# shgaurav1/DVG

Measured on AMD Instinct MI355X. Metric: predicted frames/sec at 64x64, batch 64, 10-in/10-out, higher is better.
Workload: dtype f32; 1 GPU; Moving-MNIST 64x64 rollout (generate_frames.py make_gifs sample loop), vgg_64 + lstm + GP trigger sample at i%15==0, batch 64 per GPU, 10-in/10-out; model_family=vgg, batch_per_gpu=64, n_past=10, n_future=10, parallelism=replicas x1 (no data-path collective), launch=hipGraph replay, rollouts_in_flight=3, tile_policy=energy, loop_invariant_skip_halves=hoisted, upsample_conv3x3=as transposed 4x4/s2 conv, conv3x3_deep_layers=Winograd F(4x4,3x3) / F(2x2,3x3)

## Files before the change

### dvg_amd/csrc/conv_igemm2.hip

```cpp
#include <cstdlib>
#include <type_traits>

#include "dvg_common.h"

namespace dvg {

constexpr int DVG_GEMM_WGS_PER_CU = DVG_BF16X3 ? 3 : 4;
constexpr int DVG_GEMM128_WGS = DVG_BF16X3 ? 3 : 2;
constexpr int DVG_GEMM128_GT = DVG_BF16X3 ? 2 : 4;
constexpr int DVG_GEMM_GT = 4;
constexpr int DVG_GEMM128_MIN_WGS = 4 * 768;
[[maybe_unused]] constexpr int DVG_GEMM_NT2 = 256;
constexpr int DVG_TILE16_MIN_WGS = 256;

enum { M2_CONV3 = 0, M2_CONV4S2 = 1, M2_CONVT4S2 = 2, M2_GEMM = 3 };

struct Igemm2Params {
    const float* x;
    const float* skip;
    const float* w;
    const float* scale;
    const float* shift;
    float* y;
    float* y_pool;
// ... 839 lines not shown
    if (s > 8) s = 8;
    if (s > nchunks / 4) s = nchunks / 4;
    return s < 2 ? 1 : (int)s;
}

static int gemm_images_per_wg(int tw, int nt, int NB, int Hg, int Wg, int Cout) {
#if DVG_BF16X3
    if (tw == 8 && nt == 1) {
        const long w1 = (long)(Hg / 8) * (Wg / 8) * NB * (Cout / 64), slots = 256L * DVG_GEMM_WGS_PER_CU;
        if (w1 % slots == 0 && w1 / slots >= 2 && w1 / slots <= 6 && NB % (w1 / slots) == 0) return (int)(w1 / slots);
    }
#endif
    return 1;
}

template <int MODE, int TI, int TH, int TW, int NT = 1, bool FIRST = false, bool PROJ = false>
static int launch2(Igemm2Params p, int Hg, int Wg, float* ws, long ws_floats, hipStream_t stream) {
    using C = Cfg2<MODE, TI, TH, TW, NT, FIRST, PROJ>;
    if (Hg % TH || Wg % TW || p.Cout % C::BN) return fail(DVG_ERR_SHAPE, "conv_igemm2: tile does not divide shape");
    p.tiles_y = Hg / TH;
    p.tiles_x = Wg / TW;
    p.tiles_n = (p.N + TI - 1) / TI;
    if (MODE == M2_GEMM) {
        const int ni = gemm_images_per_wg(TW, NT, p.N, Hg, Wg, p.Cout);
        p.gemm_ni = ni;
        p.tiles_n = p.N / ni;
    }
    p.nblk_n = p.Cout / C::BN;
    p.clk = g_clk;
    p.clk_cap = g_clk_cap;
    const long wgs = (long)p.tiles_y * p.tiles_x * p.tiles_n * p.nblk_n * (MODE == M2_CONVT4S2 ? 4 : 1);
    {
        const long tiles = (long)p.tiles_y * p.tiles_x * p.tiles_n;
        const double per_xcd = (double)tiles * p.nblk_n / 8.0;
        const double wb = (double)C::NTAPS * (p.C1 + p.C2) * C::BN * 4, ib = (double)C::BM * (p.C1 + p.C2) * 4;
        int best = p.nblk_n;
        double cost = 1e300;
        for (int a = 1; a <= p.nblk_n; ++a) {
            if (p.nblk_n % a) continue;
            const double share_tiles = per_xcd / a;
            if (share_tiles > (double)tiles) continue;
            const double c = a * wb + (share_tiles < 1.0 ? 1.0 : share_tiles) * ib;
            if (c < cost) { cost = c; best = a; }
        }
        p.nb_group = best;
    }
    const int nchunks = (p.C1 + p.C2) / C::KC;
    int Ho, Wo;
    if (MODE == M2_CONV3 || MODE == M2_GEMM) { Ho = p.H; Wo = p.W; }
    else if (MODE == M2_CONV4S2) { Ho = p.H >> 1; Wo = p.W >> 1; }
    else { Ho = p.H * 2; Wo = p.W * 2; }
    const long out_floats = (long)p.N * Ho * Wo * p.Cout;
    int S = (ws != nullptr && C::CAN_SPLIT) ? choose_splitk(wgs, nchunks) : 1;
    if (S > 1 && (long)S * out_floats > ws_floats) return fail(DVG_ERR_SHAPE, "conv_igemm2: split-K workspace too small");
    p.cps = (nchunks + S - 1) / S;
    p.cps = (p.cps + C::CHUNKS_PER_STAGE - 1) / C::CHUNKS_PER_STAGE * C::CHUNKS_PER_STAGE;
    S = (nchunks + p.cps - 1) / p.cps;
    p.splitk = S;
    p.ws = ws;
    float* y_pool = p.y_pool;
    float* stats = p.stats;
// ... 40 lines not shown
    return 0;
}

static int gemm_tile(int NB, int Hg, int Wg, int Cout, int* tw, int* nt) {
    int ti, th;
    if (tile2(M2_GEMM, NB, Hg, Wg, Cout, &ti, &th, tw) != 0 || ti != 1) return -1;
    *nt = 1;
    if (DVG_BF16X3 && g_tile_policy && Cout % 128 == 0 && Wg % 16 == 0 &&
        (long)NB * (Hg / 8) * (Wg / 16) * (Cout / 128) >= DVG_GEMM_NT2) {
        *tw = 16;
        *nt = 2;
    }
    return 0;
}

__global__ void pack_k16_kernel(const float* __restrict__ src, float* __restrict__ dst, int cout, int cin, int kh,
                                int kw, int transposed) {
    const long total = (long)cout * cin * kh * kw / 2;
    const int nblk = cout >> 6, taps = kh * kw;
    for (long i = blockIdx.x * (long)blockDim.x + threadIdx.x; i < total; i += (long)gridDim.x * blockDim.x) {
        const int k = (int)(i & 7) * 2;
        long r = i >> 3;
        const int co = r % cout; r /= cout;
        const int t = r % taps;
        const int chunk = r / taps;
        const int ci = chunk * 16 + k, a = t / kw, b = t % kw;
        const long j = transposed ? ((((long)ci * cout + co) * kh + (kh - 1 - a)) * kw + (kw - 1 - b))
                                  : ((((long)co * cin + ci) * kh + a) * kw + b);
        const long j1 = j + (transposed ? (long)cout * kh * kw : (long)kh * kw);
        int slot = t;
// ... 112 lines not shown
extern "C" int dvg_conv3x3_first_pair(const float* frame, const float* w0, const float* scale0, const float* shift0,
                                      const float* w1_k16, const float* scale1, const float* shift1, float* y, float* y_pool,
                                      int N, int H, int W, int Cout, int act, float slope, int y_from, void* stream) {
    DVG_REQUIRE(frame && w0 && scale0 && shift0, DVG_ERR_NULL, "dvg_conv3x3_first_pair: NULL pointer");
    DVG_REQUIRE(y_from >= 0 && y_from <= N && (y_from == 0 || y_pool != nullptr) && (y != nullptr || y_from == N), DVG_ERR_SHAPE,
                "dvg_conv3x3_first_pair: y_from=%d needs 0 <= y_from <= N, a pooled output when > 0, y unless == N", y_from);
    float* const y_biased = y ? y - (size_t)y_from * H * W * Cout : y_pool;
    Igemm2Params p{frame , nullptr, w1_k16, scale1, shift1, y_biased, y_pool, nullptr, N, H, W, 64, 0, Cout, 0,
                   act, slope, 0, 0, 0, 0, 0, 1, 0, nullptr};
    p.first_frame = frame; p.first_w = w0; p.first_scale = scale0; p.first_shift = shift0; p.first_slope = 0.2f;
    p.y_from = y_from;
    if (int e = checks2(p, "dvg_conv3x3_first_pair")) return e;
    DVG_REQUIRE(H % 8 == 0 && W % 16 == 0 && (long)N * (H / 8) * (W / 16) * (Cout / 64) >= 512, DVG_ERR_SHAPE,
                "dvg_conv3x3_first_pair: H %% 8, W %% 16 and >= 512 workgroups needed (N=%d H=%d W=%d Cout=%d)", N, H, W, Cout);
    return launch2<M2_CONV3, 1, 8, 16, 1, true>(p, H, W, nullptr, 0, (hipStream_t)stream);
}

extern "C" int dvg_conv4x4s2_bn_act_v2(const float* x, const float* w_k16, const float* scale, const float* shift,
                                       float* y, float* stats, int N, int H, int W, int Cin, int Cout, int act,
                                       float slope, float* workspace, long workspace_floats, void* stream) {
    Igemm2Params p{x, nullptr, w_k16, scale, shift, y, nullptr, stats, N, H, W, Cin, 0, Cout, 0, act, slope, 0, 0, 0, 0, 0,
                   1, 0, nullptr};
    if (int e = checks2(p, "dvg_conv4x4s2_bn_act_v2")) return e;
    DVG_REQUIRE(H % 2 == 0 && W % 2 == 0, DVG_ERR_SHAPE, "dvg_conv4x4s2_bn_act_v2: odd input");
    DVG_REQUIRE((long)N * H * W * Cin < (1L << 31), DVG_ERR_SHAPE,
                "dvg_conv4x4s2_bn_act_v2: input of %d x %d x %d x %d floats too large (32-bit offsets)", N, H, W, Cin);
    int Hg = H / 2, Wg = W / 2, ti, th, tw;
    DVG_REQUIRE(tile2(M2_CONV4S2, N, Hg, Wg, Cout, &ti, &th, &tw) == 0, DVG_ERR_SHAPE,
                "dvg_conv4x4s2_bn_act_v2: unsupported map %dx%d", H, W);
    D2(M2_CONV4S2, 1, 8, 16)
// ... 86 lines not shown
```

### dvg_amd/fused.py

```python
from __future__ import annotations

import collections
import contextlib
import functools
import os
import types
import weakref

import torch
import torch.nn as nn

from . import _derived, ops, weights
from ._derived import derived, version_key as _ver
from .ops import ACT_LRELU, ACT_NONE, ACT_SIGMOID, ACT_TANH, MODE_CONV3, MODE_CONV4S2, MODE_CONVT4S2


WINOGRAD = int(os.environ.get("DVG_WINOGRAD", "4"))
if WINOGRAD not in (0, 2, 4):
    raise RuntimeError("DVG_WINOGRAD must be 0, 2 or 4")


_WINO_MIN_C = 64
_WINO_MAX_HW = 32

# ... 85 lines not shown

BLOCKS = {
    "conv3": Block(_raw_conv3, MODE_CONV3, (0, 3, 3), 1, _dgrad_conv3),
    "conv4s2": Block(_raw_plain("conv4x4s2"), MODE_CONV4S2, (0, 4, 4), 1, _dgrad_conv4s2),
    "convT4s2": Block(_raw_convT4s2, MODE_CONVT4S2, (1, 4, 4), 0, _dgrad_convT4s2),
    "conv3_first": Block(_raw_plain("conv3x3_first"), None, (0, 3, 3), 1, None),
    "conv4s2_first": Block(_raw_plain("conv4x4s2_first"), None, (0, 4, 4), 1, None),
}


def block_weight(kind, weight, lo=None, hi=None):
    blk = BLOCKS[kind]
    return weight if blk.mode is None else weights.packed(weight, bool(blk.finish[0]), lo, hi, blk.cat)


def _skip_half(kind, skip, ps, conv=None):
    if kind == "conv3" and conv is not None and not conv.training and not torch.is_grad_enabled():
        n, c, h, w = skip.shape
        ctot = conv.weight.shape[1]
        if winograd_tile(n, c, h, w, conv.weight.shape[0]) == 4:
            return ops.conv3x3_winograd(skip, weights.winograd(conv.weight, 4, ctot - c, ctot), None, None, act=ACT_NONE)
    return BLOCKS[kind].raw(skip, None, ps, None)


_scope = types.SimpleNamespace(passes=1, groups=None, trace=None, share=None)


@contextlib.contextmanager
def _scoped(result=None, **fields):
    prev = {k: getattr(_scope, k) for k in fields}
    vars(_scope).update(fields)
    try:
        yield result
    finally:
        vars(_scope).update(prev)

# ... 275 lines not shown
                        d = ops.convT4x4s2_proj(x, weights.k4_packed(conv.weight, x.shape[1]), sc, sh,
                                                ops._last_wmat_cached(w_last, 0, 64, 9 * w_last.shape[1]), act=act, slope=slope,
                                                addend=hs[1])
                        return ops.LastProj(d, (x.shape[0], 64, 2 * x.shape[2], 2 * x.shape[3]), w_last)
                    return ops.convT4x4s2(x, None, weights.k4_packed(conv.weight, x.shape[1]), sc, sh, act=act, slope=slope,
                                          addend=hs[1])
                return ops.conv3x3(x, None, hs[0], sc, sh, upsample=upsample, act=act, slope=slope, addend=hs[1])
        if skip is None and not upsample:
            n, c, h, w = x.shape
            cout = conv.weight.shape[0]
            m = winograd_tile(n, c, h, w, cout)
            if m:
                to_v = m == 4 and not torch.is_grad_enabled() and _hand_over(next_conv, next_up, n, cout, h, w, pool)
                return ops.conv3x3_winograd(x, weights.winograd(conv.weight, m), sc, sh, act=act, slope=slope, pool=pool,
                                            to_v=to_v, y_from=y_from)
        return _from(ops.conv3x3(x, skip, weights.packed(conv.weight), sc, sh, upsample=upsample, act=act, slope=slope,
                                 pool=pool), y_from)
    return _train_block("conv3", conv, bn, x, skip, up=upsample, act=act, slope=slope, pool=pool)


def conv3_first_bn_act(conv, bn, x_nchw, *, act=ACT_LRELU, slope=0.2):
    if _needs_grad(x_nchw, conv.weight, bn.weight):
        from .autograd import conv_block_autograd
        return conv_block_autograd("conv3_first", conv, bn, x_nchw, None, act=act, slope=slope)
    if not bn.training:
        sc, sh = folded_affine(conv, bn)
        return ops.conv3x3_first(x_nchw, conv.weight, sc, sh, act=act, slope=slope)
    return _train_block("conv3_first", conv, bn, x_nchw, act=act, slope=slope)


FIRST_PAIR = True


def first_pair_applies(conv0, bn0, conv1, bn1, x_nchw) -> bool:
    if not FIRST_PAIR or bn0.training or bn1.training or _needs_grad(x_nchw, conv0.weight, bn0.weight, conv1.weight, bn1.weight):
        return False
    n, nc, h, w = x_nchw.shape
    return conv0.out_channels == 64 and conv1.in_channels == 64 and ops.first_pair_ok(n, nc, h, w, conv1.out_channels)


def conv3_first_pair(conv0, bn0, conv1, bn1, x_nchw, *, pool=False, slope=0.2, y_from=0):
    sc0, sh0 = folded_affine(conv0, bn0)
    sc1, sh1 = folded_affine(conv1, bn1)
    return ops.conv3x3_first_pair(x_nchw, weights.first_pair_taps(conv0.weight), sc0, sh0, weights.packed(conv1.weight), sc1, sh1,
                                  slope=slope, pool=pool, y_from=y_from)


def conv4s2_bn_act(conv, bn, x, *, act=ACT_LRELU, slope=0.2):
    if _needs_grad(x, conv.weight, bn.weight):
        from .autograd import conv_block_autograd
        return conv_block_autograd("conv4s2", conv, bn, x, None, act=act, slope=slope)
    if not bn.training:
        sc, sh = folded_affine(conv, bn)
        return ops.conv4x4s2(x, weights.packed(conv.weight), sc, sh, act=act, slope=slope)
    return _train_block("conv4s2", conv, bn, x, act=act, slope=slope)


def conv4s2_first_bn_act(conv, bn, x_nchw, *, act=ACT_LRELU, slope=0.2):
# ... 83 lines not shown
```

### dvg_amd/ops/__init__.py

```python
from ._core import (
    ACT_NONE, ACT_LRELU, ACT_TANH, ACT_SIGMOID, MODE_CONV3, MODE_CONV4S2, MODE_CONVT4S2, _stream, KernelTimer,
    set_timer, _run, _p, _dev_f32, nhwc_empty, is_nhwc, to_nhwc, to_nchw, tile_policy,
)
from .conv import (
    pack_conv_weight, pack_convT_weight, packed_row_floats, pack_igemm_weight, _wp_dims, unpack_conv_weight,
    unpack_convT_weight, _splitk_ws, _SPLITK_WS, evict_captured_workspaces, _stats_buf, _tile_images, SharedBlocks,
    _MAP_CACHE, shared_map, group_sum, _check_addend, conv3x3, CONV4S2_MAX_FLOATS, conv4x4s2, convT4x4s2,
    PROJ_MAX_T, convT4x4s2_proj,
)
from .winograd import (
    winograd_weight, winograd_ok, WinoV, winograd_chain_ok, winograd_up_chain_ok, winograd_pool_chain_ok,
    conv3x3_winograd, stem_up_winograd_input,
)
from .edge import (
    conv3x3_first, first_pair_ok, conv3x3_first_pair, convT3x3_last, conv4x4s2_first, convT4x4s2_last, pixel_proj,
    _SKIP_PROJ_CACHE, clear_skip_proj_cache, _cached_skip_proj, _last_wmat, _last_wmat_cached,
    precompute_skip_proj, LastProj, convT_last_two_step, eval_frames, eval_frames_finn, pairwise_frame_mse, moving_mnist_compose, clip_gather, clip_gather_aug, CLIP_MAX_SHIFT,
    mnist_scale_u8, moving_mnist_compose_u8, frame_mosaic, QUANT_TRUNC, QUANT_NEAREST,
    MOSAIC_BLACK, MOSAIC_RED, MOSAIC_GREEN, MOSAIC_SEL_NONE, MOSAIC_SEL_BEST, MOSAIC_SEL_PICK, MOSAIC_CELL_INTS,
)
from .dense import (
    gemm_nt, lstm_cell, lstm_cell_pre, lstm_cell_bwd, lstm_cell_x, stem_gemm, transpose2d, colsum, GEMM_TN_MAX_ROWS,
    gemm_tn, lstm_gates_bwd, gru_cell, gru_cell_pre, rnn_cell, gru_gates_bwd,
)
from .norm import (
    channel_stats, set_sync_bn_state, sync_bn_state, sync_partial_rows, bn_finalize, bn_act_apply, bn_act_bwd,
)
from .gp import (
    gp_predict, gp_var_norms, gp_trigger_step, gp_trigger_replay, gp_trigger_select, gp_elbo, gp_elbo_bwd,
    sum_steps, gp_step_group, gp_train_bwd,
# ... 13 lines not shown
```

### dvg_amd/ops/conv.py

```python
from __future__ import annotations

import torch

from .._derived import register
from .._lib import check, lib
from ._core import ACT_LRELU, MODE_CONV3, MODE_CONV4S2, MODE_CONVT4S2, _dev_f32, _p, _run, _stream, is_nhwc, nhwc_empty


def pack_conv_weight(w: torch.Tensor) -> torch.Tensor:
    _dev_f32(w, "pack_conv_weight")
    w = w.detach().contiguous()
    co, ci, kh, kw = w.shape
    out = torch.empty((kh * kw, co, ci), device=w.device, dtype=torch.float32)
    check(lib().dvg_pack_conv_weight(_p(w), _p(out), co, ci, kh, kw, _stream()), "pack_conv_weight")
    return out


def pack_convT_weight(w: torch.Tensor) -> torch.Tensor:
    _dev_f32(w, "pack_convT_weight")
    w = w.detach().contiguous()
    ci, co, kh, kw = w.shape
    out = torch.empty((kh * kw, co, ci), device=w.device, dtype=torch.float32)
    check(lib().dvg_pack_convT_weight(_p(w), _p(out), ci, co, kh, kw, _stream()), "pack_convT_weight")
    return out
# ... 157 lines not shown
        raise RuntimeError(f"conv3x3: packed weight {tuple(wp.shape)} does not match Cin={c1 + c2}")
    y = nhwc_empty(n, cout, h, w, x.device)
    yp = nhwc_empty(n, cout, h // 2, w // 2, x.device) if pool else None
    addend, amap, ablk = _check_addend(addend, y, pool)
    ws = _splitk_ws(MODE_CONV3, n, h, w, cin, cout, y.numel(), x.device)
    if stats:
        rows = lib().dvg_conv_stats_rows_v2(MODE_CONV3, n, h, w, cin, cout, int(pool), int(ws is not None))
    st = _stats_buf(rows, cout, x.device, _tile_images(MODE_CONV3, n, h, w, cin, cout, h, w, ws)) if stats else None
    fl, by = 2.0 * n * h * w * cout * 9 * cin, 4.0 * (x.numel() + (skip.numel() if c2 else 0) + n * h * w * cout +
                                                      wp.numel())
    _run("conv3x3_igemm", fl, by, lib().dvg_conv3x3_bn_act_v2, _p(x), _p(skip), _p(wp), _p(scale), _p(shift), _p(y),
         _p(yp), _p(st), n, h, w, c1, c2, cout, int(upsample), act, slope, _p(ws), 0 if ws is None else ws.numel(),
         _p(addend), _p(amap), ablk, _stream())
    out = (y, yp) if pool else y
    return (out, st) if stats else out


CONV4S2_MAX_FLOATS = 1 << 31


def conv4x4s2(x, wp, scale, shift, *, act=ACT_LRELU, slope=0.2, stats=False):
    _dev_f32(x, "conv4x4s2.x")
    assert is_nhwc(x)
    n, cin, h, w = x.shape
    taps, cout, cin_w = _wp_dims(wp)
    if taps != 16 or cin_w != cin:
        raise RuntimeError(f"conv4x4s2: packed weight {tuple(wp.shape)} does not match Cin={cin}")
    y = nhwc_empty(n, cout, h // 2, w // 2, x.device)
    if x.numel() >= CONV4S2_MAX_FLOATS:
        per = (CONV4S2_MAX_FLOATS - 1) // (cin * h * w)
# ... 87 lines not shown
```

### dvg_amd/ops/edge.py

```python
from __future__ import annotations

import numpy as np
import torch

from .._derived import derived, register
from .._lib import CONSTANTS, check, lib
from ._core import ACT_LRELU, ACT_SIGMOID, ACT_TANH, _dev_f32, _p, _run, _stream, is_nhwc, nhwc_empty
from .conv import SharedBlocks, _stats_buf, _wp_dims


def conv3x3_first(x_nchw, w, scale, shift, *, act=ACT_LRELU, slope=0.2, stats=False):
    _dev_f32(x_nchw, "conv3x3_first.x")
    x = x_nchw if x_nchw.is_contiguous() else x_nchw.contiguous()
    n, nc, h, wd = x.shape
    w = w.detach()
    cout = w.shape[0]
    if tuple(w.shape) != (cout, nc, 3, 3) or not w.is_contiguous():
        raise RuntimeError("conv3x3_first: weight must be contiguous (Cout,nc,3,3)")
    y = nhwc_empty(n, cout, h, wd, x.device)
    st = _stats_buf(lib().dvg_conv_first_stats_rows(3, n, h, wd), cout, x.device, 1) if stats else None
    _run("conv3x3_first", 2.0 * n * h * wd * cout * 9 * nc, 4.0 * (x.numel() + n * h * wd * cout),
         lib().dvg_conv3x3_first, _p(x), _p(w), _p(scale), _p(shift), _p(y), _p(st), n, h, wd, nc, cout, act, slope,
         _stream())
    return (y, st) if stats else y
# ... 8 lines not shown
    x = x_nchw if x_nchw.is_contiguous() else x_nchw.contiguous()
    n, nc, h, wd = x.shape
    taps, cout, cin = _wp_dims(wp1)
    w0 = w0.detach()
    if nc != 1 or tuple(w0.shape) != (9, 64) or not w0.is_contiguous() or (taps, cin) != (9, 64) or \
            not first_pair_ok(n, nc, h, wd, cout):
        raise RuntimeError(f"conv3x3_first_pair: unsupported shapes x {tuple(x.shape)} w0 {tuple(w0.shape)} wp1 {tuple(wp1.shape)}")
    if not 0 <= y_from <= n or (y_from and not pool):
        raise RuntimeError("conv3x3_first_pair: y_from needs the pooled output and 0 <= y_from <= N")
    y = nhwc_empty(n - y_from, cout, h, wd, x.device) if y_from < n else None
    yp = nhwc_empty(n, cout, h // 2, wd // 2, x.device) if pool else None
    flops = 2.0 * n * h * wd * (64 * 9 + cout * 9 * 64)
    _run("conv3x3_igemm", flops, 4.0 * (x.numel() + (0 if y is None else y.numel()) + (0 if yp is None else yp.numel()) + wp1.numel()),
         lib().dvg_conv3x3_first_pair, _p(x), _p(w0), _p(scale0), _p(shift0), _p(wp1), _p(scale1), _p(shift1), _p(y), _p(yp),
         n, h, wd, cout, act, slope, y_from, _stream(), alg_flops=flops)
    return (y, yp) if pool else y


def convT3x3_last(x, w, bias, nc, *, act=ACT_SIGMOID):
    _dev_f32(x, "convT3x3_last.x")
    assert is_nhwc(x)
    n, cin, h, wd = x.shape
    w = w.detach()
    if tuple(w.shape) != (cin, nc, 3, 3) or not w.is_contiguous():
        raise RuntimeError("convT3x3_last: weight must be contiguous (Cin,nc,3,3)")
    y = torch.empty((n, nc, h, wd), device=x.device, dtype=torch.float32)
    _run("convT3x3_last", 2.0 * n * h * wd * cin * 9 * nc, 4.0 * (x.numel() + y.numel()),
         lib().dvg_convT3x3_last, _p(x), _p(w), _p(bias), _p(y), n, h, wd, cin, nc, act, _stream())
    return y

# ... 354 lines not shown
```

### dvg_amd/weights.py

```python
from __future__ import annotations

import torch

from . import ops
from ._derived import derived


def _span(weight, lo, hi, dim):
    return (None, None, None) if lo is None or (lo == 0 and hi == weight.shape[dim]) else (lo, hi, dim)


def _sliced(weight, lo, hi, dim):
    w = weight.detach()
    if lo is not None:
        w = w[lo:hi] if dim == 0 else w[:, lo:hi]
    return w.contiguous()


def packed(weight, transposed=False, lo=None, hi=None, dim=0):
    lo, hi, dim = _span(weight, lo, hi, dim)
    return derived(weight, ("wp", transposed, lo, hi, dim), (weight,),
                   lambda: ops.pack_igemm_weight(_sliced(weight, lo, hi, dim), transposed))


def split_packed(weight, c1: int, transposed=False):
    dim = 0 if transposed else 1
    return packed(weight, transposed, 0, c1, dim), packed(weight, transposed, c1, weight.shape[dim], dim)


def winograd(weight, m, lo=None, hi=None, dgrad=False):
    lo, hi, _ = _span(weight, lo, hi, 1)

    def build():
        w = weight.detach()
        if lo is not None:
            w = w[:, lo:hi]
        if dgrad:
# ... 52 lines not shown
```

### include/dvg_hip.h

```cpp
#ifndef DVG_HIP_H
#define DVG_HIP_H

#include <stddef.h>
#include <stdint.h>

#ifdef __cplusplus
extern "C" {
#endif

#define DVG_OK 0
#define DVG_ERR_SHAPE 1
#define DVG_ERR_NULL 2
#define DVG_ERR_HIP 3
#define DVG_ERR_ALIGN 4

#define DVG_ACT_NONE 0
#define DVG_ACT_LRELU 1
#define DVG_ACT_TANH 2
#define DVG_ACT_SIGMOID 3

int dvg_abi_version(void);
const char* dvg_last_error(void);
long dvg_stream_capture_id(void* stream);

// ... 9 lines not shown
#define DVG_MODE_CONVT4S2 2
int dvg_conv_first_stats_rows(int ks, int N, int H, int W);

int dvg_mfma_mode(void);
int dvg_packed_row_floats(void);
const char* dvg_build_info(void);
void dvg_set_tile_policy(int energy);
int dvg_tile_policy(void);
int dvg_pack_conv_weight_k16(const float* w, float* w_packed, int cout, int cin, int kh, int kw, int transposed, void* stream);
int dvg_conv_splitk_v2(int mode, int N, int H, int W, int Cin, int Cout);
int dvg_conv_stats_rows_v2(int mode, int N, int H, int W, int Cin, int Cout, int pool, int with_workspace);
int dvg_conv3x3_bn_act_v2(const float* x, const float* skip, const float* w_k16, const float* scale, const float* shift, float* y,
                          float* y_pool, float* stats, int N, int H, int W, int C1, int C2, int Cout, int upsample_x, int act,
                          float slope, float* workspace, long workspace_floats, const float* addend,
                          const int* addend_map, int addend_block, void* stream);
int dvg_conv3x3_first_pair(const float* frame, const float* w0, const float* scale0, const float* shift0,
                           const float* w1_k16, const float* scale1, const float* shift1, float* y, float* y_pool,
                           int N, int H, int W, int Cout, int act, float slope,
                           int y_from ,
                           void* stream);
int dvg_conv4x4s2_bn_act_v2(const float* x, const float* w_k16, const float* scale, const float* shift, float* y, float* stats,
                            int N, int H, int W, int Cin, int Cout, int act, float slope, float* workspace, long workspace_floats,
                            void* stream);
int dvg_convT4x4s2_bn_act_v2(const float* x, const float* skip, const float* w_k16, const float* scale, const float* shift, float* y,
                             float* stats, int N, int H, int W, int C1, int C2, int Cout, int act, float slope, float* workspace,
                             long workspace_floats, const float* addend, const int* addend_map , int addend_block, void* stream);
int dvg_convT4x4s2_bn_act_proj(const float* x, const float* w_k16, const float* scale, const float* shift, const float* proj_w, float* proj_out, int T,
                               int N, int H, int W, int C1, int Cout, int act, float slope, const float* addend, const int* addend_map, int addend_block, void* stream);

int dvg_winograd_weight(const float* w_oihw, float* u_k16, int cout, int cin, int m, void* stream);
int dvg_winograd_input(const float* x, float* v, int N, int H, int W, int C, int m, int upsample, void* stream);
int dvg_gemm_batched_k16(const float* x, const float* w_k16, float* y, int NB, int H, int W, int Cin, int Cout, void* stream);
int dvg_gemm_batched_plan(int NB, int H, int W, int Cin, int Cout, int* tile_w, int* nt, int* ni);
int dvg_winograd_transform_width(long tiles, int C);
int dvg_winograd_output(const float* mm, const float* scale, const float* shift, float* y, float* y_pool, int N, int H,
                        int W, int C, int act, float slope, int m, const float* addend,
                        int y_from , void* stream);
int dvg_winograd_output_input(const float* mm, const float* scale, const float* shift, float* v_next, int N, int H, int W,
// ... 247 lines not shown
```

Before: 53270 frames/s.

## Add width-wise Winograd F(2,3) implicit-GEMM conv3x3 kernel with fused first-layer pair

Adds a bf16x3 MFMA conv3x3 kernel that applies a 1-D Winograd F(2,3) transform along the width, so each pair of output pixels uses 12 packed taps instead of 18. The input transform is done in LDS inside the kernel, and the output transform, BN, activation, addend and 2x2 max-pool are fused into the epilogue. A FIRST variant also computes the 1-channel first conv on the fly. The change adds a weight-packing kernel and Python wrappers, and moves the nb_group heuristic into a helper. The aim is fewer MFMA operations on the high-resolution 3x3 layers, at the cost of extra transform work, LDS traffic and some change in rounding.

```diff
diff --git a/dvg_amd/csrc/conv_igemm2.hip b/dvg_amd/csrc/conv_igemm2.hip
--- a/dvg_amd/csrc/conv_igemm2.hip
+++ b/dvg_amd/csrc/conv_igemm2.hip
@@ -877,6 +877,20 @@
     return 1;
 }
 
+static int choose_nb_group(long tiles, int nblk_n, double wb, double ib) {
+    const double per_xcd = (double)tiles * nblk_n / 8.0;
+    int best = nblk_n;
+    double cost = 1e300;
+    for (int a = 1; a <= nblk_n; ++a) {
+        if (nblk_n % a) continue;
+        const double share_tiles = per_xcd / a;
+        if (share_tiles > (double)tiles) continue;
+        const double c = a * wb + (share_tiles < 1.0 ? 1.0 : share_tiles) * ib;
+        if (c < cost) { cost = c; best = a; }
+    }
+    return best;
+}
+
 template <int MODE, int TI, int TH, int TW, int NT = 1, bool FIRST = false, bool PROJ = false>
 static int launch2(Igemm2Params p, int Hg, int Wg, float* ws, long ws_floats, hipStream_t stream) {
     using C = Cfg2<MODE, TI, TH, TW, NT, FIRST, PROJ>;
@@ -893,21 +907,8 @@
     p.clk = g_clk;
     p.clk_cap = g_clk_cap;
     const long wgs = (long)p.tiles_y * p.tiles_x * p.tiles_n * p.nblk_n * (MODE == M2_CONVT4S2 ? 4 : 1);
-    {
-        const long tiles = (long)p.tiles_y * p.tiles_x * p.tiles_n;
-        const double per_xcd = (double)tiles * p.nblk_n / 8.0;
-        const double wb = (double)C::NTAPS * (p.C1 + p.C2) * C::BN * 4, ib = (double)C::BM * (p.C1 + p.C2) * 4;
-        int best = p.nblk_n;
-        double cost = 1e300;
-        for (int a = 1; a <= p.nblk_n; ++a) {
-            if (p.nblk_n % a) continue;
-            const double share_tiles = per_xcd / a;
-            if (share_tiles > (double)tiles) continue;
-            const double c = a * wb + (share_tiles < 1.0 ? 1.0 : share_tiles) * ib;
-            if (c < cost) { cost = c; best = a; }
-        }
-        p.nb_group = best;
-    }
+    p.nb_group = choose_nb_group((long)p.tiles_y * p.tiles_x * p.tiles_n, p.nblk_n,
+                                 (double)C::NTAPS * (p.C1 + p.C2) * C::BN * 4, (double)C::BM * (p.C1 + p.C2) * 4);
     const int nchunks = (p.C1 + p.C2) / C::KC;
     int Ho, Wo;
     if (MODE == M2_CONV3 || MODE == M2_GEMM) { Ho = p.H; Wo = p.W; }
@@ -978,6 +979,346 @@
     return 0;
 }
 
+#if DVG_BF16X3
+struct CfgWX {
+    static constexpr int TH = 8, TP = 8, TW = 2 * TP, HH = TH + 2, HW = TW + 2, HP = HH * HW;
+    static constexpr int LD = 28, LDB = 24, WROW = DVG_WROW;
+    static constexpr int PLANE = HH * TP * LD + 8;
+    static constexpr int A_FLOATS = 4 * PLANE, B_FLOATS = 4 * 64 * LDB;
+    static constexpr int NLB = 4 * 64 * WROW / 4 / 256;
+    static constexpr int ND = (HP * 4 + 255) / 256;
+    static constexpr int D_FLOATS = ND * 64 * 16;
+    static constexpr int NX = 4 * HH * TP * 4 / 256;
+    static constexpr int FP_W = HW + 2, FP_FLOATS = (HH + 2) * FP_W;
+    static constexpr int lds_bytes(bool first) { return (A_FLOATS + B_FLOATS + D_FLOATS + (first ? FP_FLOATS : 0)) * 4; }
+    static_assert(4 * HH * TP * 4 % 256 == 0 && 4 * 64 * WROW / 4 % 256 == 0, "whole passes");
+};
+
+template <bool FIRST>
+__global__ __launch_bounds__(256, 2) void conv3_wx_kernel(const Igemm2Params p) {
+    using C = CfgWX;
+    constexpr int LD = C::LD, LDB = C::LDB, NLB = C::NLB, ND = C::ND, NX = C::NX;
+    extern __shared__ __attribute__((aligned(16))) float smem[];
+    float* const As = smem;
+    float* const Bs = As + C::A_FLOATS;
+    float* const Ds = Bs + C::B_FLOATS;
+    float* const Fp = Ds + C::D_FLOATS;
+
+    const int tid = threadIdx.x, lane = tid & 63, wave = tid >> 6;
+    const int wm = wave >> 1, wn = wave & 1, l31 = lane & 31, hh = lane >> 5;
+
+    const unsigned lid = xcd_remap(blockIdx.x, gridDim.x);
+    const int tiles_total = p.tiles_x * p.tiles_y * p.tiles_n;
+    const unsigned lr = lid / p.nb_group;
+    const int nb = (int)(lr / tiles_total) * p.nb_group + (int)(lid % p.nb_group);
+    unsigned t = lr % tiles_total;
+    const int tx_i = t % p.tiles_x; t /= p.tiles_x;
+    const int ty_i = t % p.tiles_y; t /= p.tiles_y;
+    const int n0 = (int)t, y0 = ty_i * C::TH, x0 = tx_i * C::TW, yin0 = y0 - 1, xin0 = x0 - 1, nb0 = nb * 64;
+
+    const int a_base = (wm * 32 + l31) * LD + hh * 4;
+    const int b_base = (wn * 32 + l31) * LDB + (hh ^ ((l31 >> 3) & 1)) * 4;
+
+    f32x16 acc[4];
+#pragma unroll
+    for (int f = 0; f < 4; ++f)
+#pragma unroll
+        for (int i = 0; i < 16; ++i) acc[f][i] = 0.f;
+
+    long offx[FIRST ? 1 : ND];
+    unsigned okmask = 0;
+#pragma unroll
+    for (int i = 0; i < ND; ++i) {
+        const int hp = (tid + i * 256) >> 2;
+        const int yy = yin0 + hp / C::HW, xx = xin0 + hp % C::HW;
+        const bool ok = hp < C::HP && (unsigned)yy < (unsigned)p.H && (unsigned)xx < (unsigned)p.W;
+        okmask |= ok ? (1u << i) : 0u;
+        if constexpr (!FIRST) offx[i] = ok ? (((long)n0 * p.H + yy) * p.W + xx) * p.C1 + (tid & 3) * 4 : 0;
+    }
+    const int xf = (tid >> 2) & 3, xq = tid & 3;
+    const int x_ia = xf == 0 ? 0 : (xf == 2 ? 2 : 1), x_ib = xf == 2 ? 1 : (xf == 3 ? 3 : 2);
+    const float x_sg = xf == 1 ? 1.f : -1.f;
+    const int x_pix = (tid >> 7) * C::HW + 2 * ((tid >> 4) & 7);
+    const int x_da = (x_pix + x_ia) * 16 + xq * 4, x_db = (x_pix + x_ib) * 16 + xq * 4;
+    const int x_st = xf * C::PLANE + (tid >> 4) * LD + (xq >> 1) * 4 + (xq & 1) * 2;
+
+    f32x4 fw[FIRST ? 11 : 1];
+    f32x4 ra[ND], rb[NLB];
+    auto gload_d = [&](int c0) {
+        if constexpr (FIRST) {
+            const float* w = p.first_w + c0 + (tid & 3) * 4;
+#pragma unroll
+            for (int tp = 0; tp < 9; ++tp) fw[tp] = *reinterpret_cast<const f32x4*>(w + tp * 64);
+            fw[9] = *reinterpret_cast<const f32x4*>(p.first_scale + c0 + (tid & 3) * 4);
+            fw[10] = *reinterpret_cast<const f32x4*>(p.first_shift + c0 + (tid & 3) * 4);
+        } else {
+            const float* src = p.x + c0;
+#pragma unroll
+            for (int i = 0; i < ND; ++i)
+                ra[i] = *reinterpret_cast<const f32x4*>(((okmask >> i) & 1u) ? src + offx[i] : dvg_zero_slot);
+        }
+    };
+    auto store_d = [&]() {
+        if constexpr (FIRST) {
+#pragma unroll
+            for (int i = 0; i < ND; ++i) {
+                const int hp = min((tid + i * 256) >> 2, C::HP - 1);
+                const float* f = Fp + (hp / C::HW) * C::FP_W + hp % C::HW;
+                f32x4 v = {0.f, 0.f, 0.f, 0.f};
+#pragma unroll
+                for (int tp = 0; tp < 9; ++tp) {
+                    const float px = f[(tp / 3) * C::FP_W + tp % 3];
+#pragma unroll
+                    for (int e = 0; e < 4; ++e) v[e] = fmaf(fw[tp][e], px, v[e]);
+                }
+                const float okf = (float)((okmask >> i) & 1u);
+#pragma unroll
+                for (int e = 0; e < 4; ++e) {
+                    const float a = v[e] * fw[9][e] + fw[10][e];
+                    v[e] = fmaxf(a, a * p.first_slope) * okf;
+                }
+                ra[i] = v;
+            }
+        }
+#pragma unroll
+        for (int i = 0; i < ND; ++i) reinterpret_cast<f32x4*>(Ds)[tid + i * 256] = ra[i];
+    };
+    auto gload_b = [&](int chunk, int r) {
+        const float* tile = p.w + (((size_t)chunk * (p.Cout >> 6) + nb) * 12 + r * 4) * (64 * C::WROW);
+#pragma unroll
+        for (int j = 0; j < NLB; ++j) rb[j] = reinterpret_cast<const f32x4*>(tile)[tid + j * 256];
+    };
+    auto store_b = [&]() {
+#pragma unroll
+        for (int j = 0; j < NLB; ++j) reinterpret_cast<f32x4*>(Bs)[tid + j * 256] = rb[j];
+    };
+    auto xform_read = [&](u32x2_t (&pa)[NX][3]) {
+#pragma unroll
+        for (int s = 0; s < NX; ++s) {
+            const f32x4 a = *reinterpret_cast<const f32x4*>(&Ds[x_da + s * 2 * C::HW * 16]);
+            const f32x4 b = *reinterpret_cast<const f32x4*>(&Ds[x_db + s * 2 * C::HW * 16]);
+            f32x4 v;
+#pragma unroll
+            for (int e = 0; e < 4; ++e) v[e] = fmaf(x_sg, b[e], a[e]);
+            unsigned t0, t1, t2;
+            bf16x3_split_pair(v[0], v[1], t0, t1, t2);
+            pa[s][0][0] = t0; pa[s][1][0] = t1; pa[s][2][0] = t2;
+            bf16x3_split_pair(v[2], v[3], t0, t1, t2);
+            pa[s][0][1] = t0; pa[s][1][1] = t1; pa[s][2][1] = t2;
+        }
+    };
+    auto xform_store = [&](const u32x2_t (&pa)[NX][3]) {
+#pragma unroll
+        for (int s = 0; s < NX; ++s)
+#pragma unroll
+            for (int j = 0; j < 3; ++j) *reinterpret_cast<u32x2_t*>(&As[x_st + s * 16 * LD + j * 8]) = pa[s][j];
+    };
+
+    if constexpr (FIRST) {
+        const float* fr = p.first_frame + (size_t)n0 * p.H * p.W;
+        for (int i = tid; i < C::FP_FLOATS; i += 256) {
+            const int yy = yin0 - 1 + i / C::FP_W, xx = xin0 - 1 + i % C::FP_W;
+            Fp[i] = ((unsigned)yy < (unsigned)p.H && (unsigned)xx < (unsigned)p.W) ? fr[(size_t)yy * p.W + xx] : 0.f;
+        }
+        __syncthreads();
+    }
+    gload_d(0);
+    gload_b(0, 0);
+    store_d();
+    store_b();
+    __syncthreads();
+    {
+        u32x2_t pa[NX][3];
+        xform_read(pa);
+        xform_store(pa);
+    }
+    __syncthreads();
+
+    auto stage = [&](const int chunk, auto r_c, auto next_chunk_c, auto has_next_c) __attribute__((always_inline)) {
+        constexpr int R = decltype(r_c)::value;
+        constexpr bool NEXT_CHUNK = decltype(next_chunk_c)::value, HAS_NEXT = decltype(has_next_c)::value;
+        constexpr bool LOAD_D = NEXT_CHUNK && R == 0, STORE_D = NEXT_CHUNK && R == 1, XFORM = NEXT_CHUNK && R == 2;
+        if constexpr (LOAD_D) gload_d((chunk + 1) * 16);
+        if constexpr (HAS_NEXT) gload_b(R == 2 ? chunk + 1 : chunk, (R + 1) % 3);
+        if constexpr (STORE_D) store_d();
+        u32x2_t pa[XFORM ? NX : 1][3];
+        if constexpr (XFORM) xform_read(pa);
+
+        f32x4 fa[2][3], fb[2][3];
+#pragma unroll
+        for (int j = 0; j < 3; ++j) {
+            fa[0][j] = *reinterpret_cast<const f32x4*>(&As[a_base + R * C::TP * LD + j * 8]);
+            fb[0][j] = *reinterpret_cast<const f32x4*>(&Bs[b_base + j * 8]);
+        }
+#pragma unroll
+        for (int tt = 0; tt < 4; ++tt) {
+            const int cur = tt & 1, nxt = cur ^ 1;
+            if (tt + 1 < 4) {
+#pragma unroll
+                for (int j = 0; j < 3; ++j) {
+                    fa[nxt][j] = *reinterpret_cast<const f32x4*>(&As[a_base + (tt + 1) * C::PLANE + R * C::TP * LD + j * 8]);
+                    fb[nxt][j] = *reinterpret_cast<const f32x4*>(&Bs[b_base + (tt + 1) * 64 * LDB + j * 8]);
+                }
+            }
+            if (HAS_NEXT && tt == 3) {
+                __syncthreads();
+                if constexpr (XFORM) xform_store(pa);
+                store_b();
+            }
+            auto mm = [&](int pa_, int pb_) {
+                acc[tt] = __builtin_amdgcn_mfma_f32_32x32x16_bf16(__builtin_bit_cast(bf16x8_t, fa[cur][pa_]),
+                                                                  __builtin_bit_cast(bf16x8_t, fb[cur][pb_]), acc[tt], 0, 0, 0);
+            };
+            mm(2, 0);
+            mm(1, 1);
+            mm(0, 2);
+            mm(1, 0);
+            mm(0, 1);
+            mm(0, 0);
+            constexpr int NREAD = 6, NMFMA = 6;
+            constexpr int NVMEM = (LOAD_D ? (FIRST ? 11 : ND) : 0) + (HAS_NEXT ? NLB : 0), VPT = (NVMEM + 2) / 3;
+            if (tt == 0) __builtin_amdgcn_sched_group_barrier(0x100, NREAD + (XFORM ? 2 * NX : 0) + (STORE_D && FIRST ? 9 * ND : 0), 0);
+            if (tt + 1 < 4) {
+#pragma unroll
+                for (int r = 0; r < NREAD; ++r) {
+                    __builtin_amdgcn_sched_group_barrier(0x100, 1, 0);
+                    __builtin_amdgcn_sched_group_barrier(0x008, 1, 0);
+                }
+                if (VPT > 0) __builtin_amdgcn_sched_group_barrier(0x020, VPT, 0);
+            } else if (HAS_NEXT) {
+                constexpr int NW = NLB + (XFORM ? 3 * NX : 0);
+#pragma unroll
+                for (int r = 0; r < NW; ++r) {
+                    if (r < NMFMA) __builtin_amdgcn_sched_group_barrier(0x008, 1, 0);
+                    __builtin_amdgcn_sched_group_barrier(0x200, 1, 0);
+                }
+            } else if (!HAS_NEXT) {
+                __builtin_amdgcn_sched_group_barrier(0x008, NMFMA, 0);
+            }
+        }
+        if constexpr (HAS_NEXT) __syncthreads();
+    };
+    using std::integral_constant;
+    using T_ = integral_constant<bool, true>;
+    using F_ = integral_constant<bool, false>;
+    int st = 0;
+    auto set_prio = [&]() {
+        switch (st++ & 3) {
+            case 0: __builtin_amdgcn_s_setprio(3); break;
+            case 1: __builtin_amdgcn_s_setprio(2); break;
+            case 2: __builtin_amdgcn_s_setprio(1); break;
+            default: __builtin_amdgcn_s_setprio(0); break;
+        }
+    };
+    const int nchunks = p.C1 / 16;
+    int chunk = 0;
+    for (; chunk + 1 < nchunks; ++chunk) {
+        set_prio();
+        stage(chunk, integral_constant<int, 0>{}, T_{}, T_{});
+        set_prio();
+        stage(chunk, integral_constant<int, 1>{}, T_{}, T_{});
+        set_prio();
+        stage(chunk, integral_constant<int, 2>{}, T_{}, T_{});
+    }
+    set_prio();
+    stage(chunk, integral_constant<int, 0>{}, F_{}, T_{});
+    set_prio();
+    stage(chunk, integral_constant<int, 1>{}, F_{}, T_{});
+    set_prio();
+    stage(chunk, integral_constant<int, 2>{}, F_{}, F_{});
+    __builtin_amdgcn_s_setprio(0);
+
+    const int c = nb0 + wn * 32 + l31;
+    const float sc = p.scale ? p.scale[c] : 1.f, sf = p.shift ? p.shift[c] : 0.f;
+    const bool want_y = !FIRST || n0 >= p.y_from;
+    float* const yb = p.y + (size_t)n0 * p.H * p.W * p.Cout + c;
+    float* const pb = p.y_pool ? p.y_pool + (size_t)n0 * (p.H >> 1) * (p.W >> 1) * p.Cout + c : nullptr;
+    const float* ab = nullptr;
+    if (p.addend) ab = p.addend + (size_t)(addend_image(p.add_map, p.add_B, n0)) * p.H * p.W * p.Cout + c;
+    auto epilogue = [&](auto act_c) {
+        constexpr int ACT = decltype(act_c)::value;
+        float v[2][16];
+#pragma unroll
+        for (int reg = 0; reg < 16; ++reg) {
+            v[0][reg] = (acc[0][reg] + acc[1][reg]) + acc[2][reg];
+            v[1][reg] = (acc[1][reg] - acc[2][reg]) - acc[3][reg];
+        }
+#pragma unroll
+        for (int reg = 0; reg < 16; ++reg) {
+            const int m = wm * 32 + (reg & 3) + 8 * (reg >> 2) + 4 * hh;
+            const int off = ((y0 + (m >> 3)) * p.W + x0 + 2 * (m & 7)) * p.Cout;
+#pragma unroll
+            for (int e = 0; e < 2; ++e) {
+                float u = v[e][reg];
+                if (ab != nullptr) u += ab[off + e * p.Cout];
+                u = u * sc + sf;
+                if constexpr (ACT == DVG_ACT_LRELU) u = u > 0.f ? u : u * p.slope;
+                else if constexpr (ACT != DVG_ACT_NONE) u = apply_act(u, p.act, p.slope);
+                v[e][reg] = u;
+                if (want_y) yb[off + e * p.Cout] = u;
+            }
+        }
+        if (pb != nullptr) {
+#pragma unroll
+            for (int reg = 0; reg < 16; ++reg) {
+                if (((reg >> 2) & 1) == 0) {
+                    const int m = wm * 32 + (reg & 3) + 8 * (reg >> 2) + 4 * hh;
+                    const float mx = fmaxf(fmaxf(v[0][reg], v[1][reg]), fmaxf(v[0][reg + 4], v[1][reg + 4]));
+                    pb[(((y0 + (m >> 3)) >> 1) * (p.W >> 1) + (x0 >> 1) + (m & 7)) * p.Cout] = mx;
+                }
+            }
+        }
+    };
+    if (p.act == DVG_ACT_LRELU) epilogue(std::integral_constant<int, DVG_ACT_LRELU>{});
+    else if (p.act == DVG_ACT_NONE) epilogue(std::integral_constant<int, DVG_ACT_NONE>{});
+    else epilogue(std::integral_constant<int, -1>{});
+}
+
+template <bool FIRST>
+static int launch_wx(Igemm2Params p, hipStream_t stream) {
+    using C = CfgWX;
+    p.tiles_y = p.H / C::TH;
+    p.tiles_x = p.W / C::TW;
+    p.tiles_n = p.N;
+    p.nblk_n = p.Cout / 64;
+    const long tiles = (long)p.tiles_y * p.tiles_x * p.tiles_n;
+    p.nb_group = choose_nb_group(tiles, p.nblk_n, 12.0 * p.C1 * 64 * 4, (double)C::TH * C::TW * p.C1 * 4);
+    static bool attr_set = false;
+    if (!attr_set) {
+        hipError_t e = hipFuncSetAttribute(reinterpret_cast<const void*>(&conv3_wx_kernel<FIRST>),
+                                           hipFuncAttributeMaxDynamicSharedMemorySize, C::lds_bytes(FIRST));
+        if (e != hipSuccess) return fail(DVG_ERR_HIP, "hipFuncSetAttribute: %s", hipGetErrorString(e));
+        attr_set = true;
+    }
+    hipLaunchKernelGGL((conv3_wx_kernel<FIRST>), dim3((unsigned)(tiles * p.nblk_n)), dim3(256), C::lds_bytes(FIRST), stream, p);
+    return check_launch("conv3_wx");
+}
+#endif
+
+__global__ void pack_wx_kernel(const float* __restrict__ src, float* __restrict__ dst, int cout, int cin) {
+    const long total = (long)cout * cin * 12 / 2;
+    const int nblk = cout >> 6;
+    for (long i = blockIdx.x * (long)blockDim.x + threadIdx.x; i < total; i += (long)gridDim.x * blockDim.x) {
+        const int k = (int)(i & 7) * 2;
+        long r = i >> 3;
+        const int co = r % cout; r /= cout;
+        const int tap = r % 12;
+        const int chunk = r / 12;
+        const int row = tap >> 2, f = tap & 3;
+        float u[2];
+#pragma unroll
+        for (int e = 0; e < 2; ++e) {
+            const float* g = src + (((long)co * cin + chunk * 16 + k + e) * 3 + row) * 3;
+            if (f == 0) u[e] = g[0];
+            else if (f == 1) u[e] = ((g[0] + g[1]) + g[2]) * 0.5f;
+            else if (f == 2) u[e] = ((g[0] - g[1]) + g[2]) * 0.5f;
+            else u[e] = g[2];
+        }
+        wrow_store_pair(dst, (((size_t)chunk * nblk + (co >> 6)) * 12 + tap) * 64 + (co & 63), co & 63, k, u[0], u[1]);
+    }
+    wrow_drain();
+}
+
 __global__ void pack_k16_kernel(const float* __restrict__ src, float* __restrict__ dst, int cout, int cin, int kh,
                                 int kw, int transposed) {
     const long total = (long)cout * cin * kh * kw / 2;
@@ -1120,6 +1461,73 @@
     DVG_REQUIRE(H % 8 == 0 && W % 16 == 0 && (long)N * (H / 8) * (W / 16) * (Cout / 64) >= 512, DVG_ERR_SHAPE,
                 "dvg_conv3x3_first_pair: H %% 8, W %% 16 and >= 512 workgroups needed (N=%d H=%d W=%d Cout=%d)", N, H, W, Cout);
     return launch2<M2_CONV3, 1, 8, 16, 1, true>(p, H, W, nullptr, 0, (hipStream_t)stream);
+}
+
+extern "C" int dvg_pack_conv_weight_wx(const float* w, float* w_packed, int cout, int cin, void* stream) {
+    DVG_REQUIRE(w && w_packed, DVG_ERR_NULL, "dvg_pack_conv_weight_wx: NULL pointer");
+    DVG_REQUIRE(cout > 0 && cout % 64 == 0 && cin > 0 && cin % 16 == 0, DVG_ERR_SHAPE,
+                "dvg_pack_conv_weight_wx: Cin must be a multiple of 16, Cout of 64");
+    DVG_REQUIRE(aligned16(w_packed), DVG_ERR_ALIGN, "dvg_pack_conv_weight_wx: w_packed must be 16-byte aligned");
+    const long total = (long)cout * cin * 12 / 2;
+    hipLaunchKernelGGL(pack_wx_kernel, dim3(grid_for(total, 256, 4096)), dim3(256), 0, (hipStream_t)stream, w, w_packed, cout, cin);
+    return check_launch("dvg_pack_conv_weight_wx");
+}
+
+static int checks_wx(const Igemm2Params& p, const char* who) {
+    DVG_REQUIRE(p.N > 0 && p.H > 0 && p.W > 0, DVG_ERR_SHAPE, "%s: empty shape", who);
+    DVG_REQUIRE(p.C1 > 0 && p.C1 % 16 == 0 && p.C2 == 0 && p.skip == nullptr && !p.upsample, DVG_ERR_SHAPE,
+                "%s: Cin=%d must be a multiple of 16; no concat operand, no upsampling", who, p.C1 + p.C2);
+    DVG_REQUIRE(p.Cout > 0 && p.Cout % 64 == 0, DVG_ERR_SHAPE, "%s: Cout=%d must be a multiple of 64", who, p.Cout);
+    DVG_REQUIRE(p.H % 8 == 0 && p.W % 16 == 0, DVG_ERR_SHAPE, "%s: H=%d must be a multiple of 8, W=%d of 16", who, p.H, p.W);
+    DVG_REQUIRE((long)p.H * p.W * p.Cout < (1L << 31), DVG_ERR_SHAPE, "%s: image of %d x %d x %d floats too large", who, p.H, p.W, p.Cout);
+    DVG_REQUIRE(aligned16(p.x) && aligned16(p.w) && aligned16(p.y) && aligned16(p.y_pool) && aligned16(p.addend), DVG_ERR_ALIGN,
+                "%s: pointers must be 16-byte aligned", who);
+    DVG_REQUIRE(p.act >= DVG_ACT_NONE && p.act <= DVG_ACT_SIGMOID, DVG_ERR_SHAPE, "%s: bad act", who);
+    DVG_REQUIRE(DVG_BF16X3 != 0, DVG_ERR_SHAPE, "%s: the f32-MFMA build has no WX kernel", who);
+    return DVG_OK;
+}
+
+extern "C" int dvg_conv3x3_bn_act_wx(const float* x, const float* skip, const float* w_wx, const float* scale,
+                                     const float* shift, float* y, float* y_pool, int N, int H, int W, int C1, int C2,
+                                     int Cout, int upsample_x, int act, float slope, const float* addend,
+                                     const int* addend_map, int addend_block, void* stream) {
+    const char* who = "dvg_conv3x3_bn_act_wx";
+    DVG_REQUIRE(x && w_wx && y, DVG_ERR_NULL, "%s: x/w/y must not be NULL", who);
+    Igemm2Params p{x, skip, w_wx, scale, shift, y, y_pool, nullptr, N, H, W, C1, C2, Cout, upsample_x ? 1 : 0, act, slope,
+                   0, 0, 0, 0, 0, 1, 0, nullptr};
+    p.addend = addend;
+    p.add_map = addend ? addend_map : nullptr;
+    p.add_B = addend_block;
+    DVG_REQUIRE(p.add_map == nullptr || (addend_block > 0 && N % addend_block == 0), DVG_ERR_SHAPE, "%s: addend_block must divide N", who);
+    DVG_REQUIRE(addend == nullptr || y_pool == nullptr, DVG_ERR_SHAPE, "%s: addend excludes the pooled output", who);
+    if (int e = checks_wx(p, who)) return e;
+#if DVG_BF16X3
+    return launch_wx<false>(p, (hipStream_t)stream);
+#else
+    return DVG_ERR_SHAPE;
+#endif
+}
+
+extern "C" int dvg_conv3x3_first_pair_wx(const float* frame, const float* w0, const float* scale0, const float* shift0,
+                                         const float* w1_wx, const float* scale1, const float* shift1, float* y, float* y_pool,
+                                         int N, int H, int W, int Cout, int act, float slope, int y_from, void* stream) {
+    const char* who = "dvg_conv3x3_first_pair_wx";
+    DVG_REQUIRE(frame && w0 && scale0 && shift0 && w1_wx, DVG_ERR_NULL, "%s: NULL pointer", who);
+    DVG_REQUIRE(y_from >= 0 && y_from <= N && (y_from == 0 || y_pool != nullptr) && (y != nullptr || y_from == N), DVG_ERR_SHAPE,
+                "%s: y_from=%d needs 0 <= y_from <= N, a pooled output when > 0, y unless == N", who, y_from);
+    DVG_REQUIRE(aligned16(w0) && aligned16(scale0) && aligned16(shift0) && aligned16(y), DVG_ERR_ALIGN,
+                "%s: pointers must be 16-byte aligned", who);
+    float* const y_biased = y ? y - (size_t)y_from * H * W * Cout : y_pool;
+    Igemm2Params p{frame , nullptr, w1_wx, scale1, shift1, y_biased, y_pool, nullptr, N, H, W, 64, 0, Cout, 0,
+                   act, slope, 0, 0, 0, 0, 0, 1, 0, nullptr};
+    p.first_frame = frame; p.first_w = w0; p.first_scale = scale0; p.first_shift = shift0; p.first_slope = 0.2f;
+    p.y_from = y_from;
+    if (int e = checks_wx(p, who)) return e;
+#if DVG_BF16X3
+    return launch_wx<true>(p, (hipStream_t)stream);
+#else
+    return DVG_ERR_SHAPE;
+#endif
 }
 
 extern "C" int dvg_conv4x4s2_bn_act_v2(const float* x, const float* w_k16, const float* scale, const float* shift,
diff --git a/dvg_amd/fused.py b/dvg_amd/fused.py
--- a/dvg_amd/fused.py
+++ b/dvg_amd/fused.py
@@ -123,12 +123,24 @@
     return weight if blk.mode is None else weights.packed(weight, bool(blk.finish[0]), lo, hi, blk.cat)
 
 
+CONV3_WX = True
+CONV3_WX_MIN_WGS = 256
+
+
+def conv3_wx_applies(n, cin, h, w, cout, *modules) -> bool:
+    return (CONV3_WX and not torch.is_grad_enabled() and not any(m.training for m in modules)
+            and ops.lib().dvg_tile_policy() == 1 and cin == 64 and w >= 64 and ops.wx_ok(n, cin, h, w, cout)
+            and ops.wx_workgroups(n, h, w, cout) >= CONV3_WX_MIN_WGS)
+
+
 def _skip_half(kind, skip, ps, conv=None):
     if kind == "conv3" and conv is not None and not conv.training and not torch.is_grad_enabled():
         n, c, h, w = skip.shape
         ctot = conv.weight.shape[1]
         if winograd_tile(n, c, h, w, conv.weight.shape[0]) == 4:
             return ops.conv3x3_winograd(skip, weights.winograd(conv.weight, 4, ctot - c, ctot), None, None, act=ACT_NONE)
+        if conv3_wx_applies(n, c, h, w, conv.weight.shape[0], conv):
+            return ops.conv3x3_wx(skip, weights.wx(conv.weight, ctot - c, ctot), None, None, act=ACT_NONE)
     return BLOCKS[kind].raw(skip, None, ps, None)
 
 
@@ -434,6 +446,8 @@
                 to_v = m == 4 and not torch.is_grad_enabled() and _hand_over(next_conv, next_up, n, cout, h, w, pool)
                 return ops.conv3x3_winograd(x, weights.winograd(conv.weight, m), sc, sh, act=act, slope=slope, pool=pool,
                                             to_v=to_v, y_from=y_from)
+            if conv3_wx_applies(n, c, h, w, cout, conv, bn):
+                return _from(ops.conv3x3_wx(x, weights.wx(conv.weight), sc, sh, act=act, slope=slope, pool=pool), y_from)
         return _from(ops.conv3x3(x, skip, weights.packed(conv.weight), sc, sh, upsample=upsample, act=act, slope=slope,
                                  pool=pool), y_from)
     return _train_block("conv3", conv, bn, x, skip, up=upsample, act=act, slope=slope, pool=pool)
@@ -462,6 +476,10 @@
 def conv3_first_pair(conv0, bn0, conv1, bn1, x_nchw, *, pool=False, slope=0.2, y_from=0):
     sc0, sh0 = folded_affine(conv0, bn0)
     sc1, sh1 = folded_affine(conv1, bn1)
+    n, _, h, w = x_nchw.shape
+    if conv3_wx_applies(n, 64, h, w, conv1.out_channels, conv0, bn0, conv1, bn1):
+        return ops.conv3x3_first_pair_wx(x_nchw, weights.first_pair_taps(conv0.weight), sc0, sh0, weights.wx(conv1.weight), sc1, sh1,
+                                         slope=slope, pool=pool, y_from=y_from)
     return ops.conv3x3_first_pair(x_nchw, weights.first_pair_taps(conv0.weight), sc0, sh0, weights.packed(conv1.weight), sc1, sh1,
                                   slope=slope, pool=pool, y_from=y_from)
 
diff --git a/dvg_amd/ops/__init__.py b/dvg_amd/ops/__init__.py
--- a/dvg_amd/ops/__init__.py
+++ b/dvg_amd/ops/__init__.py
@@ -4,6 +4,7 @@
 )
 from .conv import (
     pack_conv_weight, pack_convT_weight, packed_row_floats, pack_igemm_weight, _wp_dims, unpack_conv_weight,
+    pack_wx_weight, wx_ok, wx_workgroups, conv3x3_wx,
     unpack_convT_weight, _splitk_ws, _SPLITK_WS, evict_captured_workspaces, _stats_buf, _tile_images, SharedBlocks,
     _MAP_CACHE, shared_map, group_sum, _check_addend, conv3x3, CONV4S2_MAX_FLOATS, conv4x4s2, convT4x4s2,
     PROJ_MAX_T, convT4x4s2_proj,
@@ -13,7 +14,7 @@
     conv3x3_winograd, stem_up_winograd_input,
 )
 from .edge import (
-    conv3x3_first, first_pair_ok, conv3x3_first_pair, convT3x3_last, conv4x4s2_first, convT4x4s2_last, pixel_proj,
+    conv3x3_first, first_pair_ok, conv3x3_first_pair, conv3x3_first_pair_wx, convT3x3_last, conv4x4s2_first, convT4x4s2_last, pixel_proj,
     _SKIP_PROJ_CACHE, clear_skip_proj_cache, _cached_skip_proj, _last_wmat, _last_wmat_cached,
     precompute_skip_proj, LastProj, convT_last_two_step, eval_frames, eval_frames_finn, pairwise_frame_mse, moving_mnist_compose, clip_gather, clip_gather_aug, CLIP_MAX_SHIFT,
     mnist_scale_u8, moving_mnist_compose_u8, frame_mosaic, QUANT_TRUNC, QUANT_NEAREST,
diff --git a/dvg_amd/ops/conv.py b/dvg_amd/ops/conv.py
--- a/dvg_amd/ops/conv.py
+++ b/dvg_amd/ops/conv.py
@@ -195,6 +195,42 @@
          _p(addend), _p(amap), ablk, _stream())
     out = (y, yp) if pool else y
     return (out, st) if stats else out
+
+
+def pack_wx_weight(w: torch.Tensor) -> torch.Tensor:
+    _dev_f32(w, "pack_wx_weight")
+    w = w.detach().contiguous()
+    co, ci, kh, kw = w.shape
+    if (kh, kw) != (3, 3):
+        raise RuntimeError(f"pack_wx_weight: a 3x3 kernel is needed, got {kh}x{kw}")
+    out = torch.empty((ci // 16, 12, co, packed_row_floats()), device=w.device, dtype=torch.float32)
+    check(lib().dvg_pack_conv_weight_wx(_p(w), _p(out), co, ci, _stream()), "pack_wx")
+    return out
+
+
+def wx_ok(n, cin, h, w, cout) -> bool:
+    return cin % 16 == 0 and cout % 64 == 0 and h % 8 == 0 and w % 16 == 0 and lib().dvg_mfma_mode() == 1
+
+
+def wx_workgroups(n, h, w, cout) -> int:
+    return n * (h // 8) * (w // 16) * (cout // 64)
+
+
+def conv3x3_wx(x, wp, scale, shift, *, act=ACT_LRELU, slope=0.2, pool=False, addend=None):
+    _dev_f32(x, "conv3x3_wx.x")
+    assert is_nhwc(x), "conv3x3_wx: x must be NHWC in memory"
+    n, c1, h, w = x.shape
+    taps, cout, cin = _wp_dims(wp)
+    if taps != 12 or cin != c1:
+        raise RuntimeError(f"conv3x3_wx: packed weight {tuple(wp.shape)} does not match Cin={c1}")
+    y = nhwc_empty(n, cout, h, w, x.device)
+    yp = nhwc_empty(n, cout, h // 2, w // 2, x.device) if pool else None
+    addend, amap, ablk = _check_addend(addend, y, pool)
+    alg = 2.0 * n * h * w * cout * 9 * cin
+    by = 4.0 * (x.numel() + n * h * w * cout + wp.numel())
+    _run("conv3x3_igemm", alg * 12 / 18, by, lib().dvg_conv3x3_bn_act_wx, _p(x), None, _p(wp), _p(scale), _p(shift), _p(y),
+         _p(yp), n, h, w, c1, 0, cout, 0, act, slope, _p(addend), _p(amap), ablk, _stream(), alg_flops=alg)
+    return (y, yp) if pool else y
 
 
 CONV4S2_MAX_FLOATS = 1 << 31
diff --git a/dvg_amd/ops/edge.py b/dvg_amd/ops/edge.py
--- a/dvg_amd/ops/edge.py
+++ b/dvg_amd/ops/edge.py
@@ -46,6 +46,26 @@
     _run("conv3x3_igemm", flops, 4.0 * (x.numel() + (0 if y is None else y.numel()) + (0 if yp is None else yp.numel()) + wp1.numel()),
          lib().dvg_conv3x3_first_pair, _p(x), _p(w0), _p(scale0), _p(shift0), _p(wp1), _p(scale1), _p(shift1), _p(y), _p(yp),
          n, h, wd, cout, act, slope, y_from, _stream(), alg_flops=flops)
+    return (y, yp) if pool else y
+
+
+def conv3x3_first_pair_wx(x_nchw, w0, scale0, shift0, wx1, scale1, shift1, *, act=ACT_LRELU, slope=0.2, pool=False, y_from=0):
+    _dev_f32(x_nchw, "conv3x3_first_pair_wx.x")
+    x = x_nchw if x_nchw.is_contiguous() else x_nchw.contiguous()
+    n, nc, h, wd = x.shape
+    taps, cout, cin = _wp_dims(wx1)
+    w0 = w0.detach()
+    if nc != 1 or tuple(w0.shape) != (9, 64) or not w0.is_contiguous() or (taps, cin) != (12, 64) or h % 8 or wd % 16:
+        raise RuntimeError(f"conv3x3_first_pair_wx: unsupported shapes x {tuple(x.shape)} w0 {tuple(w0.shape)} wx1 {tuple(wx1.shape)}")
+    if not 0 <= y_from <= n or (y_from and not pool):
+        raise RuntimeError("conv3x3_first_pair_wx: y_from needs the pooled output and 0 <= y_from <= N")
+    y = nhwc_empty(n - y_from, cout, h, wd, x.device) if y_from < n else None
+    yp = nhwc_empty(n, cout, h // 2, wd // 2, x.device) if pool else None
+    alg = 2.0 * n * h * wd * (64 * 9 + cout * 9 * 64)
+    flops = 2.0 * n * h * wd * (64 * 9 + cout * 6 * 64)
+    _run("conv3x3_igemm", flops, 4.0 * (x.numel() + (0 if y is None else y.numel()) + (0 if yp is None else yp.numel()) + wx1.numel()),
+         lib().dvg_conv3x3_first_pair_wx, _p(x), _p(w0), _p(scale0), _p(shift0), _p(wx1), _p(scale1), _p(shift1), _p(y), _p(yp),
+         n, h, wd, cout, act, slope, y_from, _stream(), alg_flops=alg)
     return (y, yp) if pool else y
 
 
diff --git a/dvg_amd/weights.py b/dvg_amd/weights.py
--- a/dvg_amd/weights.py
+++ b/dvg_amd/weights.py
@@ -21,6 +21,11 @@
     lo, hi, dim = _span(weight, lo, hi, dim)
     return derived(weight, ("wp", transposed, lo, hi, dim), (weight,),
                    lambda: ops.pack_igemm_weight(_sliced(weight, lo, hi, dim), transposed))
+
+
+def wx(weight, lo=None, hi=None):
+    lo, hi, dim = _span(weight, lo, hi, 1)
+    return derived(weight, ("wx", lo, hi), (weight,), lambda: ops.pack_wx_weight(_sliced(weight, lo, hi, dim)))
 
 
 def split_packed(weight, c1: int, transposed=False):
diff --git a/include/dvg_hip.h b/include/dvg_hip.h
--- a/include/dvg_hip.h
+++ b/include/dvg_hip.h
@@ -47,14 +47,14 @@
                           float* y_pool, float* stats, int N, int H, int W, int C1, int C2, int Cout, int upsample_x, int act,
                           float slope, float* workspace, long workspace_floats, const float* addend,
                           const int* addend_map, int addend_block, void* stream);
-int dvg_conv3x3_first_pair(const float* frame, const float* w0, const float* scale0, const float* shift0,
-                           const float* w1_k16, const float* scale1, const float* shift1, float* y, float* y_pool,
-                           int N, int H, int W, int Cout, int act, float slope,
-                           int y_from ,
-                           void* stream);
+int dvg_conv3x3_first_pair(const float* frame, const float* w0, const float* scale0, const float* shift0, const float* w1_k16,
+                           const float* scale1, const float* shift1, float* y, float* y_pool, int N, int H, int W, int Cout, int act, float slope,
+                           int y_from , void* stream);
+int dvg_pack_conv_weight_wx(const float* w, float* w_packed, int cout, int cin, void* stream);
+int dvg_conv3x3_bn_act_wx(const float* x, const float* skip, const float* w_wx, const float* scale, const float* shift, float* y, float* y_pool, int N, int H, int W, int C1, int C2, int Cout, int upsample_x, int act, float slope, const float* addend, const int* addend_map, int addend_block, void* stream);
+int dvg_conv3x3_first_pair_wx(const float* frame, const float* w0, const float* scale0, const float* shift0, const float* w1_wx, const float* scale1, const float* shift1, float* y, float* y_pool, int N, int H, int W, int Cout, int act, float slope, int y_from, void* stream);
 int dvg_conv4x4s2_bn_act_v2(const float* x, const float* w_k16, const float* scale, const float* shift, float* y, float* stats,
-                            int N, int H, int W, int Cin, int Cout, int act, float slope, float* workspace, long workspace_floats,
-                            void* stream);
+                            int N, int H, int W, int Cin, int Cout, int act, float slope, float* workspace, long workspace_floats, void* stream);
 int dvg_convT4x4s2_bn_act_v2(const float* x, const float* skip, const float* w_k16, const float* scale, const float* shift, float* y,
                              float* stats, int N, int H, int W, int C1, int C2, int Cout, int act, float slope, float* workspace,
                              long workspace_floats, const float* addend, const int* addend_map , int addend_block, void* stream);
```

Result: faster. 53890 frames/s (median of 6 runs) (+1.2%).
